# huggingface/parler-tts

Hardware: AMD Instinct MI355X
Metric: audio-seconds/sec (whole node) + p50 time-to-first-token, Mini-v1 bs=1/32 (higher is better)
Workload: dtype bf16; 1 GPU; parler-tts-mini-v1 bf16 bs=1/GPU greedy, 64 description + 32 prompt tokens, 860 frames = 9.985 s audio/utterance (868 decoder passes, hipGraph decode, DAC on-GPU); global_batch=1, frames=860, parallelism=utterance-sharded x1, weights broadcast once

## Files before the change

### parler_tts_amd/_native.py

```python
from __future__ import annotations

import ctypes as C
import os
from typing import Optional

PTTS_F32, PTTS_BF16 = 0, 1
PTTS_OK, PTTS_E_INVALID, PTTS_E_HIP, PTTS_E_MISSING, PTTS_E_CAPACITY, PTTS_E_UNSUPPORTED = 0, -1, -2, -3, -4, -5

_HERE = os.path.dirname(os.path.abspath(__file__))
LIB_PATH = os.path.join(_HERE, "libptts_hip.so")


class NativeLibraryError(RuntimeError):
    pass


class PttsConfig(C.Structure):
    _fields_ = [
        ("hidden_size", C.c_int32), ("num_layers", C.c_int32), ("num_heads", C.c_int32), ("ffn_dim", C.c_int32),
        ("num_codebooks", C.c_int32), ("vocab_size", C.c_int32), ("max_positions", C.c_int32), ("rope", C.c_int32),
        ("rope_theta", C.c_float), ("pad_token_id", C.c_int32), ("eos_token_id", C.c_int32), ("bos_token_id", C.c_int32),
        ("dtype", C.c_int32), ("max_batch", C.c_int32), ("max_ctx", C.c_int32), ("max_enc", C.c_int32),
        ("max_prompt", C.c_int32), ("device", C.c_int32), ("num_kv_heads", C.c_int32), ("num_cross_kv_heads", C.c_int32),
        ("weights_fp8", C.c_int32), ("kv_fp8", C.c_int32),
# ... 71 lines not shown
    "ptts_dac_debug_latents": (C.c_int, [_VP, C.POINTER(_VP)]),
    "ptts_t5_create": (C.c_int, [C.POINTER(PttsT5Config), C.POINTER(_VP)]),
    "ptts_t5_destroy": (None, [_VP]),
    "ptts_t5_load_weight": (C.c_int, [_VP, C.c_char_p, _VP, _I32, _I64P, _I32, _VP]),
    "ptts_t5_weights_ready": (C.c_int, [_VP]),
    "ptts_t5_encode": (C.c_int, [_VP, _VP, _VP, _I32, _I32, _VP, _VP]),
    "ptts_t5_relative_bucket": (C.c_int32, [_I32, _I32, _I32]),
    "ptts_t5_debug_graph_nodes": (C.c_int, [_VP, C.POINTER(_I32)]),
    "ptts_dac_debug_decode_upto": (C.c_int, [_VP, _VP, _I32, _I32, _I32, _VP, C.POINTER(_VP), C.POINTER(_I32), C.POINTER(_VP), C.POINTER(_I32), C.POINTER(_I32)]),
}

SESSION_SYMBOLS = {
    "ptts_admit_rows": (C.c_int, [_VP, _I32, C.POINTER(_I32), _VP, _VP, _VP, _VP, C.POINTER(_I32), _I32, C.POINTER(C.POINTER(PttsGenParams)), _VP]),
}

_lib: Optional[C.CDLL] = None


def load_library(path: Optional[str] = None) -> C.CDLL:
    global _lib
    if _lib is not None and path is None:
        return _lib
    import torch

    p = path or os.environ.get("PTTS_LIB", LIB_PATH)
    if not os.path.exists(p):
        raise NativeLibraryError(
            f"{p} not found: the HIP library is required (there is no CPU fallback). "
            "Build it with `python -c 'import __graft_entry__ as g; g.build()'`.")
    try:
        lib = C.CDLL(p)
    except OSError as e:
        raise NativeLibraryError(f"failed to load {p}: {e}") from e
    for name, (res, args) in list(SYMBOLS.items()) + list(SESSION_SYMBOLS.items()):
        try:
            fn = getattr(lib, name)
        except AttributeError as e:
            raise NativeLibraryError(f"{p} does not export {name}") from e
        fn.restype = res
        fn.argtypes = args
    if lib.ptts_abi_version() != ABI_VERSION:
        raise NativeLibraryError(f"ABI version mismatch: library {lib.ptts_abi_version()} != binding {ABI_VERSION}")
    if path is None:
        _lib = lib
    return lib


_hip: Optional[C.CDLL] = None

# ... 25 lines not shown
```

### parler_tts_amd/csrc/ptts_lm.hip

```cpp
#include <array>
#include <map>
#include <set>
#include <string>
#include <type_traits>
#include <vector>

#include "ptts_common.h"
#include "ptts_lm_kernels.h"
#include "ptts_gemv.h"
#include "ptts_strip_w8.h"
#include "ptts_gemm_launch.h"
#include "ptts_tail_launch.h"

thread_local std::string g_ptts_err;
int ptts_fail(int code, const char* fmt, ...) {
  char buf[1024];
  va_list ap;
  va_start(ap, fmt);
  vsnprintf(buf, sizeof(buf), fmt, ap);
  va_end(ap);
  g_ptts_err = buf;
  return code;
}
extern "C" const char* ptts_last_error(void) { return g_ptts_err.c_str(); }
// ... 61 lines not shown
  DevGen* gen = nullptr;
  ptts_gen_params gp;
  int B = 0, N = 0, P = 0;
  bool prefilled = false;
  bool h_ready = false;
  int lnproj = -1;
  int fuse_qa_max = 3;
  int last_graph_nodes = 0;
  bool fuse_qa = true;
  int fuse_x = -1;
  int fuse_x_nur = 2;
  float* xpart = nullptr;
  float* h2 = nullptr;
  bool fuse_xq = true;
  int lnproj_g = 0;
  int xattn_g = 0;
  bool xattn_g_ok = false;
  bool xattn_groups = true;
  int kv_ub = 0;
  int kv_bound = 0;
  std::map<long long, hipGraphExec_t> graphs;
  int* host_pinned = nullptr;
  bool session = false;
  int session_max_length = 0;
  int* row_maxlen = nullptr;
  SlotGen* slot_gen = nullptr;
  float* h_adm = nullptr;
  KvLayer* kv_layers_rows = nullptr;
  float* h_adm_rows = nullptr;
  AdmitMoveLayer* move_layers = nullptr;
// ... 53 lines not shown
}

inline void* at(void* p, size_t off) { return static_cast<char*>(p) + off; }

#ifdef PTTS_TIMING
#define PTTS_DBG_STAMP(args, on_, node_) (args).dbg = (e->dbg_stamps && (on_)) ? e->dbg_stamps + (node_) * 48 : nullptr
#else
#define PTTS_DBG_STAMP(args, on_, node_) do { } while (0)
#endif

int launch_status(const char* what) {
  hipError_t err = hipGetLastError();
  return err == hipSuccess ? PTTS_OK : ptts_fail(PTTS_E_HIP, "%s launch failed: %s", what, hipGetErrorString(err));
}

template <typename WT, int EPI>
int launch_lnproj(const ptts_engine* e, LnProjArgs p, hipStream_t st, int g) {
  constexpr int KT = Elem<WT>::KT;
  const int H = p.K;
  p.invK = 1.0f / (float)H;
  const int mg = p.M < g ? p.M : g;
  const size_t sh = (size_t)mg * (H * sizeof(WT) + 16) + 8 * 1024;
  const dim3 grid(p.N / 64, (p.M + g - 1) / g);
  const bool u16 = ((H / KT) / 2) % 16 == 0;
#define PTTS_LNPROJ_ONE(UW, NF4, G)                                                                                   \
  do {                                                                                                                \
    static PttsPerDeviceOnce attr_once;                                                                               \
    const int attr_dev = PttsPerDeviceOnce::device();                                                                 \
    if (sh > 64 * 1024 && attr_once.need(attr_dev)) {                                                                 \
      hipError_t ea = hipFuncSetAttribute(reinterpret_cast<const void*>(&lnproj_fused_kernel<WT, UW, NF4, G, EPI>),  \
                                          hipFuncAttributeMaxDynamicSharedMemorySize, 160 * 1024);                    \
      if (ea != hipSuccess) return ptts_fail(PTTS_E_HIP, "hipFuncSetAttribute(max dynamic LDS) failed: %s", hipGetErrorString(ea)); \
      attr_once.done(attr_dev);                                                                                       \
    }                                                                                                                 \
    ptts_klaunch(lnproj_fused_kernel<WT, UW, NF4, G, EPI>, grid, dim3(512), sh, st, p);                      \
  } while (0)
#define PTTS_LNPROJ_LAUNCH(UW, NF4)                                                                                   \
  do {                                                                                                                \
// ... 212 lines not shown

template <typename WT>
int strip_path(const ptts_engine* e, FwdView v, bool prefill, int Q, hipStream_t st) {
  const ptts_config& c = e->cfg;
  const int H = c.hidden_size, F = c.ffn_dim, nh = c.num_heads, B = v.B;
  const int nkv = e->nkv, nkc = e->nkc, Hkv = nkv * 64, QKV = H + 2 * Hkv;
  const int M = B * Q;
  const bool big = M > 8;
  const int dec = prefill ? 0 : 1;
  const float scale = 1.0f / sqrtf((float)(H / nh));
  const int S_used = prefill ? 1 : e->S_self;
  const bool lns = e->use_lns && !prefill && M > 8 && M <= 32;
  const int fo = (M > 8 && (!prefill || M <= 256)) ? 1 : 0;
  const int KT = Elem<WT>::KT;
  const int lnproj = e->lnproj >= 0 ? e->lnproj : 3;
  const int lnproj_g = e->lnproj_g > 0 ? e->lnproj_g : (M <= 40 ? 8 : 16);
  const bool lnproj_ok = lnproj > 0 && (!prefill || M <= 40) && M > 8 && !e->w8_strips && (H == 1024 || H == 1536) && ((H / KT) / 2) % 8 == 0 && QKV % 64 == 0 && F % 64 == 0;
  const int prefill_attn_mode = getenv("PTTS_PREFILL_ATTN") ? atoi(getenv("PTTS_PREFILL_ATTN")) : 3;
  const bool prefill_attn = prefill_attn_mode != 0;
  const bool kv_in_qkv = prefill && lnproj_ok && !c.rope && !e->L[0].ks_self;
  const bool kv_in_gemm = prefill && !kv_in_qkv && !lnproj_ok && M > 256 && !c.rope && !e->L[0].ks_self;
#define PTTS_DBG_BIG(args, l_, k_) PTTS_DBG_STAMP(args, !prefill && M > 8, (size_t)(l_) * 7 + (k_))
  for (int l = 0; l < c.num_layers; ++l) {
    const LayerW& w = e->L[l];
    void *const k_self = at(w.k_self, v.self_off), *const v_self = at(w.v_self, v.self_off);
    if (lnproj_ok) {
      LnProjArgs p = {};
      PTTS_DBG_BIG(p, l, 0);
      p.W = w.qkv; p.x = v.h; p.x_ld = H; p.gamma = w.ln1_g; p.beta = w.ln1_b; p.K = H; p.out = e->qkv; p.out_ld = QKV; p.M = M; p.N = QKV;
      if (kv_in_qkv) { p.kcache = k_self; p.vcache = v_self; p.kv_Q = Q; p.kv_cap = c.max_ctx; p.kv_heads = nkv; p.kv_H = H; }
      PTTS_TRY((launch_lnproj<WT, EPI_STORE>(e, p, st, lnproj_g)));
    } else {
      GemmArgs g = {}; g.decode = dec;
      g.W = w.qkv; g.W8 = w.qkv_p8; g.wscale = w.qkv_sc; g.x = v.h; g.x_ld = H; g.x_row_mul = 1; g.gamma = w.ln1_g; g.beta = w.ln1_b;
      g.out = e->qkv; g.out_ld = QKV; g.M = M; g.N = QKV; g.K = H; g.x_fo = fo;
      if (kv_in_gemm) { g.kcache = k_self; g.vcache = v_self; g.kv_rows_per_b = Q; g.kv_cap = c.max_ctx; g.nheads = nkv; g.kv_col0 = H; }
      PTTS_TRY((gemm_with_prologue<WT, PRO_LN, EPI_STORE>(e, g, st)));
    }
    if (prefill && !kv_in_qkv && !kv_in_gemm) {
      bool done8 = false;
      if constexpr (sizeof(WT) == 2) {
        if (w.ks_self) {
          hipLaunchKernelGGL((kv_append_kernel<WT, true>), dim3(Q, nkv, B), dim3(64), 0, st, e->qkv + H, e->qkv + H + Hkv, QKV, k_self, v_self, c.max_ctx,
                             Q, nkv, c.rope ? e->rope_cos : nullptr, c.rope ? e->rope_sin : nullptr, w.ks_self, w.vs_self);
          done8 = true;
        }
// ... 23 lines not shown
      }
    }
    if (!prefill && (M <= 8 || (e->xattn_groups && M <= 256)) && (H / KT) % 16 == 0 && (H == 512 || H == 1024 || H == 1536)) {
      XAttnArgs x = {};
      x.W = w.cq; x.x = v.h; x.x_ld = H; x.x_row_mul = 1; x.x_row_off = 0; x.gamma = w.ln2_g; x.beta = w.ln2_b; x.K = H;
      x.invK = 1.0f / (float)H; x.kcache = at(w.k_cross, v.cross_off); x.vcache = at(w.v_cross, v.cross_off); x.cap = c.max_enc; x.cur_len = v.cur_len; x.dims = e->dims;
      x.mask = v.enc_mask; x.mask_ld = c.max_enc; x.cos = c.rope ? e->rope_cos : nullptr; x.sin = c.rope ? e->rope_sin : nullptr;
      x.out = e->xw; x.B = M; x.nheads = nh; x.kv_heads = nkc; x.n_rep = nh / nkc; x.scale = scale; x.out_fo = fo;
      PTTS_DBG_BIG(x, l, 3);
      const int gsz = M <= 8 ? 8 : (e->xattn_g ? e->xattn_g : (e->xattn_g_ok ? (M <= 32 ? 2 : (M <= 64 ? 4 : 8)) : 8));
      launch_xattn_fused<WT>(x, gsz, st);
    } else {
    if (prefill && lnproj_ok) {
      LnProjArgs p = {};
      p.W = w.cq; p.x = v.h; p.x_ld = H; p.gamma = w.ln2_g; p.beta = w.ln2_b; p.K = H; p.out = e->qc; p.out_ld = H; p.M = M; p.N = H;
      PTTS_TRY((launch_lnproj<WT, EPI_STORE>(e, p, st, lnproj_g)));
    } else
    {
      GemmArgs g = {}; g.decode = dec;
      g.W = w.cq; g.x = v.h; g.x_ld = H; g.x_row_mul = 1; g.gamma = w.ln2_g; g.beta = w.ln2_b;
      g.out = e->qc; g.out_ld = H; g.M = M; g.N = H; g.K = H; g.x_fo = fo;
      if (lns) g.lnstat = e->lnstat;
      PTTS_TRY((gemm_with_prologue<WT, PRO_LN, EPI_STORE>(e, g, st)));
    }
    {
      AttnArgs a = cross_attn_args(e, v, w, Q, prefill, fo);
      a.hostP = v.P; a.hostN = v.N;
      if (prefill && prefill_attn) PTTS_TRY((launch_prefill_attn<WT>(a, B, st, prefill_attn_mode)));
      else PTTS_TRY((launch_attn<WT>(a, B, st, prefill ? 4 : e->cross_waves)));
    }
    }
// ... 6 lines not shown
      PTTS_TRY((launch_gemm<WT, PRO_COPY, EPI_RESID>(g, st)));
    }
    {
      GemmArgs g = {}; g.decode = dec;
      g.W = w.fc1; g.W8 = w.fc1_p8; g.wscale = w.fc1_sc; g.x = v.h; g.x_ld = H; g.x_row_mul = 1; g.gamma = w.ln3_g; g.beta = w.ln3_b;
      g.out_ld = F; g.M = M; g.N = F; g.K = H;
      GemmArgs g2 = {}; g2.decode = dec;
      g2.W = w.fc2; g2.W8 = w.fc2_p8; g2.wscale = w.fc2_sc; g2.x_ld = F; g2.x_row_mul = 1; g2.out = v.h; g2.out_ld = H; g2.M = M; g2.N = H; g2.K = F;
      if (big) {
        g.out = reinterpret_cast<float*>(e->xw2); g.x_fo = fo; g.out_fo = fo;
        if (lns) g.lnstat = e->lnstat;
        if (lnproj_ok && (lnproj >= 3 || (lnproj == 2 && M > 32))) {
          LnProjArgs p = {};
          p.W = w.fc1; p.x = v.h; p.x_ld = H; p.gamma = w.ln3_g; p.beta = w.ln3_b; p.K = H; p.out = e->xw2; p.out_ld = F; p.out_fo = fo; p.M = M; p.N = F;
          PTTS_DBG_BIG(p, l, 5);
          PTTS_TRY((launch_lnproj<WT, EPI_GELU_WT>(e, p, st, lnproj_g)));
        } else
        PTTS_TRY((gemm_with_prologue<WT, PRO_LN, EPI_GELU_WT>(e, g, st)));
        g2.x = reinterpret_cast<const float*>(e->xw2); g2.x_fo = fo;
        PTTS_DBG_BIG(g2, l, 6);
        PTTS_TRY((launch_gemm<WT, PRO_COPY, EPI_RESID>(g2, st)));
      } else {
        g.out = e->ffn;
        PTTS_TRY((launch_gemm<WT, PRO_LN, EPI_GELU>(g, st)));
        g2.x = e->ffn;
        PTTS_TRY((launch_gemm<WT, PRO_PLAIN, EPI_RESID>(g2, st)));
      }
    }
  }
  {
    GemmArgs g = {}; g.decode = dec;
// ... 109 lines not shown
           {"encoder_attn.out_proj.weight", w.co, w.co_rm, w.co_p8, w.co_sc, H, H, 0},
           {"fc1.weight", w.fc1, w.fc1_rm, w.fc1_p8, w.fc1_sc, F, H, 0},
           {"fc2.weight", w.fc2, w.fc2_rm, w.fc2_p8, w.fc2_sc, H, F, 0},
           {"self_attn_layer_norm.weight", w.ln1_g, nullptr, nullptr, nullptr, H, -1, 0}, {"self_attn_layer_norm.bias", w.ln1_b, nullptr, nullptr, nullptr, H, -1, 0},
           {"encoder_attn_layer_norm.weight", w.ln2_g, nullptr, nullptr, nullptr, H, -1, 0}, {"encoder_attn_layer_norm.bias", w.ln2_b, nullptr, nullptr, nullptr, H, -1, 0},
           {"final_layer_norm.weight", w.ln3_g, nullptr, nullptr, nullptr, H, -1, 0}, {"final_layer_norm.bias", w.ln3_b, nullptr, nullptr, nullptr, H, -1, 0}}};
}

void read_env_switches(ptts_engine* e) {
  if (const char* ev = getenv("PTTS_FUSE_X")) e->fuse_x = atoi(ev) ? 1 : 0;
  if (const char* ev = getenv("PTTS_FUSE_X_NUR")) { const int v = atoi(ev); if (v == 2 || v == 4) e->fuse_x_nur = v; }
  e->fuse_qa = !(getenv("PTTS_NO_FUSE_QA") && atoi(getenv("PTTS_NO_FUSE_QA")));
  if (const char* ev = getenv("PTTS_FUSE_QA_MAX")) e->fuse_qa_max = std::max(1, std::min(GV_MAX_ROWS, atoi(ev)));
  e->fuse_xq = !(getenv("PTTS_NO_FUSE_XQ") && atoi(getenv("PTTS_NO_FUSE_XQ")));
  if (const char* ev = getenv("PTTS_LNPROJ")) e->lnproj = std::max(0, std::min(3, atoi(ev)));
  if (const char* ev = getenv("PTTS_LNPROJ_G")) e->lnproj_g = atoi(ev) == 4 ? 4 : (atoi(ev) == 16 ? 16 : (atoi(ev) == 8 ? 8 : 0));
  if (const char* ev = getenv("PTTS_XATTN_G")) { const int g = atoi(ev); if (g == 2 || g == 4 || g == 8) e->xattn_g = e->xattn_g_ok ? g : 8; }
  e->xattn_groups = !(getenv("PTTS_NO_XATTN_GROUPS") && atoi(getenv("PTTS_NO_XATTN_GROUPS")));
}

hipStream_t pick_stream(ptts_engine*, void* s) { return reinterpret_cast<hipStream_t>(s); }

}

extern "C" int ptts_engine_create(const ptts_config* cfg, ptts_engine** out) {
  PTTS_CHECK(cfg && out, PTTS_E_INVALID, "null argument");
  const ptts_config& c = *cfg;
  PTTS_CHECK(c.hidden_size > 0 && c.num_heads > 0 && c.hidden_size % c.num_heads == 0, PTTS_E_INVALID, "hidden_size %d not divisible by num_heads %d", c.hidden_size, c.num_heads);
  PTTS_CHECK(c.hidden_size / c.num_heads == 64, PTTS_E_UNSUPPORTED, "head_dim must be 64 (Mini/Large v1), got %d", c.hidden_size / c.num_heads);
  PTTS_CHECK(c.dtype == PTTS_F32 || c.dtype == PTTS_BF16, PTTS_E_INVALID, "dtype must be PTTS_F32 or PTTS_BF16");
  PTTS_CHECK(c.hidden_size % 32 == 0 && c.ffn_dim % 32 == 0 && c.vocab_size % 16 == 0, PTTS_E_UNSUPPORTED,
// ... 135 lines not shown
  A(e->alloc(&e->qc, std::max(rows, enc_rows) * H));
  const size_t part_rows = std::max(rows * (size_t)e->S_self, (size_t)c.max_batch * 5) + 9;
  A(e->alloc(&e->part, part_rows * H));
  A(e->alloc(&e->stats, part_rows * nh * 2));
  A(e->alloc(&e->xpart, (size_t)nh * H));
  A(e->alloc(&e->h2, (size_t)H));
  A(e->alloc(&e->ffn, std::max(rows * F, rows * (size_t)H)));
  A(e->alloc(&e->logits, (size_t)c.max_batch * K * V));
  A(e->alloc(&e->sort_buf, 16));
  A(e->alloc_bytes(&e->xw, (rows + 16) * H * es));
  A(e->alloc_bytes(&e->xw2, std::max((rows + 16) * F, enc_rows * (size_t)H) * es));
  A(e->alloc(&e->lnstat, (size_t)c.max_batch * (H / 16) * 2 + 16));
  e->use_lns = H == 1024 || H == 1536;
  e->xattn_g_ok = (H == 1024 && ((H / (c.dtype == PTTS_BF16 ? 32 : 16)) / 2) % 16 == 0) || H == 1536;
  read_env_switches(e);
  A(e->alloc(&e->prefix, (size_t)c.max_batch * K * c.max_ctx));
  e->ids_ld = c.max_ctx + 8;
  A(e->alloc(&e->ids, (size_t)c.max_batch * K * e->ids_ld));
  A(e->alloc(&e->cur_len, c.max_batch)); A(e->alloc(&e->unfinished, (size_t)c.max_batch * K));
  A(e->alloc(&e->has_eos, (size_t)c.max_batch * K)); A(e->alloc(&e->first_unf, c.max_batch));
  A(e->alloc(&e->enc_mask, enc_rows + 64));
  A(e->alloc(&e->prompt_mask, rows));
  A(e->alloc(&e->dims, 1)); A(e->alloc(&e->gen, 1));
#undef A
  if (hipHostMalloc((void**)&e->host_pinned, ((size_t)c.max_batch * (K + 1) + 16) * 4) != hipSuccess) return fail(ptts_fail(PTTS_E_HIP, "hipHostMalloc failed"));
#ifdef PTTS_TIMING
  {
    const size_t n = (size_t)(c.num_layers + 1) * 7 * 48;
    rc = e->alloc(&e->dbg_stamps, n);
    if (rc != PTTS_OK) return fail(rc);
// ... 577 lines not shown
#ifdef PTTS_TIMING
extern "C" int ptts_debug_stamps(ptts_engine* e, long long** stamps_dev, int32_t* layers) {
  PTTS_CHECK(e && stamps_dev && layers, PTTS_E_INVALID, "null argument");
  *stamps_dev = e->dbg_stamps;
  *layers = e->cfg.num_layers;
  return PTTS_OK;
}
#endif

extern "C" int ptts_debug_graph_nodes(ptts_engine* e, int32_t* nodes) {
  PTTS_CHECK(e && nodes, PTTS_E_INVALID, "null argument");
  *nodes = e->last_graph_nodes;
  return PTTS_OK;
}

extern "C" int ptts_debug_hidden(ptts_engine* e, float** hidden_dev, int32_t* rows) {
  PTTS_CHECK(e && hidden_dev && rows, PTTS_E_INVALID, "null argument");
  *hidden_dev = e->h;
  *rows = e->B;
  return PTTS_OK;
}
```

### parler_tts_amd/csrc/ptts_lm_kernels.h

```cpp
#pragma once
#include "ptts_common.h"

struct DevDims {
  int P;
  int N;
  int max_length;
  int T_prefix;
  const long long* prefix;
  int prefix_ld;
};
struct DevGen {
  int max_length, min_new_tokens, do_sample, top_k, use_eos_gate;
  float temperature, top_p;
  unsigned long long seed;
};

template <typename ST> __device__ __forceinline__ float load_as_f32(const ST* p);
template <> __device__ __forceinline__ float load_as_f32<float>(const float* p) { return *p; }
template <> __device__ __forceinline__ float load_as_f32<bf16_t>(const bf16_t* p) { return bf16_to_f32(*p); }
template <typename DT> __device__ __forceinline__ void store_from_f32(DT* p, float v);
template <> __device__ __forceinline__ void store_from_f32<float>(float* p, float v) { *p = v; }
template <> __device__ __forceinline__ void store_from_f32<bf16_t>(bf16_t* p, float v) { *p = f32_to_bf16(v); }

template <typename WT, typename ST>
// ... 1785 lines not shown
  KDBG0(X)                                                                                                                              \
  KF(X, const void*, W)                                                                       \
  KF(X, const float*, x)                                                                               \
  KF(X, const float*, gamma) KF(X, const float*, beta) KF(X, void*, out)                                                              \
  KF(X, int, x_ld)                                                                                                                      \
  KF(X, int, K)                                                                                          \
  KF(X, int, M) KF(X, int, N) KTAIL(X, LnProjArgs)
struct LnProjArgs {
  PTTS_KMEMBERS(LnProjArgs)
  float invK;
  int out_ld;
  int out_fo;
  int kv_Q;
  void* kcache;
  void* vcache;
  int kv_cap, kv_heads, kv_H, kv_pad_;
  PTTS_DBG_FIELD
};
PTTS_KLAUNCH(LnProjArgs)

template <typename WT, int UW, int NF4, int G, int EPI>
__global__ void __launch_bounds__(512) lnproj_fused_kernel(PTTS_KPARAMS(LnProjArgs)) {
  PTTS_STAMP0();
  PTTS_KJOIN(LnProjArgs, a)
  constexpr int KT = Elem<WT>::KT, NWV = 8;
  static_assert(G <= 2 * NWV, "at most two rows per wave");
  extern __shared__ __attribute__((aligned(16))) char smem_raw[];
  const int lane = threadIdx.x & 63, wave = threadIdx.x >> 6;
  const int b0 = blockIdx.y * G, nb = min(G, a.M - b0), nbmax = min(G, a.M);
  const int row_bytes = a.K * (int)sizeof(WT) + 16;
  char* s_x = smem_raw;
  float* s_red = reinterpret_cast<float*>(smem_raw + (size_t)nbmax * row_bytes);
  const int nfrag = a.K / KT;
  const int strip = blockIdx.x * 4 + (wave >> 1);
  const int per = nfrag >> 1;
  const int t0 = (wave & 1) * per, t1 = t0 + per;
  const uint4* Wp = reinterpret_cast<const uint4*>(a.W) + (size_t)strip * nfrag * 64 + lane;
  const int q4 = lane >> 4, j = lane & 15;
  uint4 afr[UW];
  PTTS_WSTAMP(a, 0);
  if constexpr (G > NWV) {
    if (wave < nb) {
      const bool two = wave + NWV < nb;
      const float* xr0 = a.x + (size_t)(b0 + wave) * a.x_ld;
      const float* xr1 = a.x + (size_t)(b0 + (two ? wave + NWV : wave)) * a.x_ld;
      float4 v0[NF4], v1[NF4], g[NF4], bt[NF4];
#pragma unroll
      for (int i = 0; i < NF4; ++i) { v0[i] = *reinterpret_cast<const float4*>(xr0 + (lane + 64 * i) * 4); v1[i] = *reinterpret_cast<const float4*>(xr1 + (lane + 64 * i) * 4); }
#pragma unroll
      for (int i = 0; i < NF4; ++i) {
        g[i] = *reinterpret_cast<const float4*>(a.gamma + (lane + 64 * i) * 4);
        bt[i] = *reinterpret_cast<const float4*>(a.beta + (lane + 64 * i) * 4);
      }
      __builtin_amdgcn_sched_barrier(0);
      __builtin_amdgcn_s_barrier();
#pragma unroll
      for (int uu = 0; uu < UW; ++uu) afr[uu] = ld_nt16(Wp + (size_t)(t0 + uu) * 64);
      __builtin_amdgcn_sched_barrier(0);
      auto norm_row = [&](float4 (&v)[NF4], char* row) __attribute__((always_inline)) {
        const float c = __int_as_float(__builtin_amdgcn_readfirstlane(__float_as_int(v[0].x)));
        float s1 = 0.f, s2 = 0.f;
#pragma unroll
        for (int i = 0; i < NF4; ++i) {
          const float d0 = v[i].x - c, d1 = v[i].y - c, d2 = v[i].z - c, d3 = v[i].w - c;
          s1 += (d0 + d1) + (d2 + d3);
          s2 += (d0 * d0 + d1 * d1) + (d2 * d2 + d3 * d3);
        }
        s1 = wave_sum(s1);
        s2 = wave_sum(s2);
        const float dm = s1 * a.invK, mean = c + dm;
        const float rstd = rsqrtf(fmaxf(s2 * a.invK - dm * dm, 0.f) + 1e-5f);
#pragma unroll
        for (int i = 0; i < NF4; ++i)
          lds_store4<WT>(row, (lane + 64 * i) * 4, (v[i].x - mean) * rstd * g[i].x + bt[i].x, (v[i].y - mean) * rstd * g[i].y + bt[i].y,
                         (v[i].z - mean) * rstd * g[i].z + bt[i].z, (v[i].w - mean) * rstd * g[i].w + bt[i].w);
      };
      PTTS_WSTAMP(a, 1);
      norm_row(v0, s_x + (size_t)wave * row_bytes);
      if (two) norm_row(v1, s_x + (size_t)(wave + NWV) * row_bytes);
      PTTS_WSTAMP(a, 2);
    } else {
      __builtin_amdgcn_sched_barrier(0);
      __builtin_amdgcn_s_barrier();
#pragma unroll
      for (int uu = 0; uu < UW; ++uu) afr[uu] = ld_nt16(Wp + (size_t)(t0 + uu) * 64);
      __builtin_amdgcn_sched_barrier(0);
    }
  } else
  if (wave < nb) {
    const int m = b0 + wave;
    const float* xr = a.x + (size_t)m * a.x_ld;
    float4 v[NF4], g[NF4], bt[NF4];
#pragma unroll
    for (int i = 0; i < NF4; ++i) v[i] = *reinterpret_cast<const float4*>(xr + (lane + 64 * i) * 4);
#pragma unroll
    for (int i = 0; i < NF4; ++i) {
      g[i] = *reinterpret_cast<const float4*>(a.gamma + (lane + 64 * i) * 4);
      bt[i] = *reinterpret_cast<const float4*>(a.beta + (lane + 64 * i) * 4);
    }
    __builtin_amdgcn_sched_barrier(0);
    __builtin_amdgcn_s_barrier();
#pragma unroll
    for (int uu = 0; uu < UW; ++uu) afr[uu] = ld_nt16(Wp + (size_t)(t0 + uu) * 64);
    __builtin_amdgcn_sched_barrier(0);
    PTTS_WSTAMP(a, 1);
    const float c = __int_as_float(__builtin_amdgcn_readfirstlane(__float_as_int(v[0].x)));
    float s1 = 0.f, s2 = 0.f;
#pragma unroll
    for (int i = 0; i < NF4; ++i) {
      const float d0 = v[i].x - c, d1 = v[i].y - c, d2 = v[i].z - c, d3 = v[i].w - c;
      s1 += (d0 + d1) + (d2 + d3);
      s2 += (d0 * d0 + d1 * d1) + (d2 * d2 + d3 * d3);
    }
    s1 = wave_sum(s1);
    s2 = wave_sum(s2);
    const float dm = s1 * a.invK, mean = c + dm;
    const float rstd = rsqrtf(fmaxf(s2 * a.invK - dm * dm, 0.f) + 1e-5f);
    char* row = s_x + (size_t)wave * row_bytes;
#pragma unroll
    for (int i = 0; i < NF4; ++i)
      lds_store4<WT>(row, (lane + 64 * i) * 4, (v[i].x - mean) * rstd * g[i].x + bt[i].x, (v[i].y - mean) * rstd * g[i].y + bt[i].y,
                     (v[i].z - mean) * rstd * g[i].z + bt[i].z, (v[i].w - mean) * rstd * g[i].w + bt[i].w);
    PTTS_WSTAMP(a, 2);
  } else {
    __builtin_amdgcn_sched_barrier(0);
    __builtin_amdgcn_s_barrier();
#pragma unroll
    for (int uu = 0; uu < UW; ++uu) afr[uu] = ld_nt16(Wp + (size_t)(t0 + uu) * 64);
    __builtin_amdgcn_sched_barrier(0);
  }
  __syncthreads();
  PTTS_WSTAMP(a, 3);
  const char* brow = s_x + (size_t)min(j, nb - 1) * row_bytes + (size_t)q4 * 16;
  f32x4 acc = f32x4{0.f, 0.f, 0.f, 0.f}, acc2 = f32x4{0.f, 0.f, 0.f, 0.f};
  for (int tb = t0; tb < t1; tb += UW) {
    if (tb != t0) {
#pragma unroll
      for (int uu = 0; uu < UW; ++uu) afr[uu] = ld_nt16(Wp + (size_t)(tb + uu) * 64);
    }
#pragma unroll
    for (int uh = 0; uh < UW; uh += 8) {
      uint4 bfr[8];
#pragma unroll
      for (int uu = 0; uu < 8; ++uu) bfr[uu] = *reinterpret_cast<const uint4*>(brow + (size_t)(tb + uh + uu) * (KT * sizeof(WT)));
#pragma unroll
      for (int uu = 0; uu < 8; ++uu) {
        if (uu & 1) acc2 = MfmaStep<WT>::run(afr[uh + uu], bfr[uu], acc2);
        else acc = MfmaStep<WT>::run(afr[uh + uu], bfr[uu], acc);
      }
    }
  }
  PTTS_WSTAMP(a, 4);
  *reinterpret_cast<f32x4*>(s_red + ((size_t)wave * 64 + lane) * 4) = acc + acc2;
  __syncthreads();
  PTTS_WSTAMP(a, 5);
  if (wave < 4 && j < nb) {
    const f32x4 rr = *reinterpret_cast<const f32x4*>(s_red + ((size_t)(2 * wave) * 64 + lane) * 4) +
                     *reinterpret_cast<const f32x4*>(s_red + ((size_t)(2 * wave + 1) * 64 + lane) * 4);
    const int m = b0 + j, n = (blockIdx.x * 4 + wave) * 16 + q4 * 4;
    if (EPI == EPI_STORE) {
      *reinterpret_cast<float4*>(reinterpret_cast<float*>(a.out) + (size_t)m * a.out_ld + n) = make_float4(rr[0], rr[1], rr[2], rr[3]);
      if (a.kcache && n >= a.kv_H) {
        const int Hkv = a.kv_heads * 64, nn = n - a.kv_H, isv = nn >= Hkv, n2 = isv ? nn - Hkv : nn;
        const int head = n2 >> 6, d = n2 & 63, bu = m / a.kv_Q, pos = m - bu * a.kv_Q;
        WT* dst = reinterpret_cast<WT*>(isv ? a.vcache : a.kcache) + (((size_t)bu * a.kv_heads + head) * a.kv_cap + pos) * 64 + d;
#pragma unroll
        for (int e = 0; e < 4; ++e) store_from_f32<WT>(dst + e, rr[e]);
      }
    } else {
      act_store4<WT>(reinterpret_cast<WT*>(a.out), m, n, a.out_ld, a.out_fo, gelu_erf(rr[0]), gelu_erf(rr[1]), gelu_erf(rr[2]), gelu_erf(rr[3]));
    }
  }
}

template <typename WT, bool W8> struct RmRow {
  static __device__ __forceinline__ void ld8(const void* W, const float* sc, int row, int K, int k, float (&o)[8]) {
    if constexpr (W8) {
      const uint2 v = *reinterpret_cast<const uint2*>(reinterpret_cast<const uint8_t*>(W) + (size_t)row * K + k);
      const float s = sc[row];
      const auto a = __builtin_amdgcn_cvt_pk_f32_fp8((int)v.x, false), b = __builtin_amdgcn_cvt_pk_f32_fp8((int)v.x, true);
      const auto c = __builtin_amdgcn_cvt_pk_f32_fp8((int)v.y, false), d = __builtin_amdgcn_cvt_pk_f32_fp8((int)v.y, true);
      o[0] = a[0] * s; o[1] = a[1] * s; o[2] = b[0] * s; o[3] = b[1] * s; o[4] = c[0] * s; o[5] = c[1] * s; o[6] = d[0] * s; o[7] = d[1] * s;
    } else {
      const WT* p = reinterpret_cast<const WT*>(W) + (size_t)row * K + k;
#pragma unroll
      for (int e = 0; e < 8; ++e) o[e] = Elem<WT>::ld(p + e);
// ... 607 lines not shown
```

### parler_tts_amd/engine.py

```python
from __future__ import annotations

import ctypes as C
import math
from typing import Dict, Iterable, Optional, Tuple

import torch

from . import _native as N
from .quant import is_fp8_matrix


def _stream_ptr(stream: Optional["torch.cuda.Stream"] = None, device=None) -> C.c_void_p:
    s = stream if stream is not None else torch.cuda.current_stream(device)
    return C.c_void_p(s.cuda_stream)


def _shape_arr(t: torch.Tensor):
    return (C.c_int64 * t.dim())(*t.shape)


def rope_tables(head_dim: int, theta: float, num_positions: int) -> Tuple[torch.Tensor, torch.Tensor]:
    inv_freq = 1.0 / (theta ** (torch.arange(0, head_dim, 2, dtype=torch.int64).float() / head_dim))
    pos = torch.arange(num_positions, dtype=torch.int64).float()
    freqs = (inv_freq[:, None] @ pos[None, :]).transpose(0, 1)
# ... 113 lines not shown
        self.B, self.P = B, P
        self._keep = keep

    def first_token_sync(self):
        N.check(self.lib.ptts_first_token_sync(self._h), "ptts_first_token_sync")

    def first_token_times(self) -> Tuple[float, float]:
        pre, tail = C.c_float(), C.c_float()
        N.check(self.lib.ptts_first_token_times(self._h, C.byref(pre), C.byref(tail)), "ptts_first_token_times")
        return float(pre.value), float(tail.value)

    def graph_nodes(self) -> int:
        n = C.c_int32()
        N.check(self.lib.ptts_debug_graph_nodes(self._h, C.byref(n)), "ptts_debug_graph_nodes")
        return int(n.value)

    def set_audio_prefix(self, codes: Optional[torch.Tensor]):
        if codes is None or codes.shape[-1] == 0:
            N.check(self.lib.ptts_set_audio_prefix(self._h, C.c_void_p(), 1, 0, _stream_ptr(device=self.device)), "ptts_set_audio_prefix")
            return
        codes = codes.to(self.device, torch.int64).reshape(-1, codes.shape[-1]).contiguous()
        if codes.shape[0] % self.K:
            raise ValueError(f"audio prefix rows {codes.shape[0]} not a multiple of num_codebooks {self.K}")
        N.check(self.lib.ptts_set_audio_prefix(self._h, C.c_void_p(codes.data_ptr()), codes.shape[0] // self.K, codes.shape[1], _stream_ptr(device=self.device)),
                "ptts_set_audio_prefix")
        self._keep_prefix = codes

    def decode_steps(self, n: int):
        N.check(self.lib.ptts_decode_steps(self._h, int(n), _stream_ptr(device=self.device)), "ptts_decode_steps")

# ... 449 lines not shown
```

Measured before the change: 20.63 audio-seconds/sec.

## Make lnproj kernel loop over weight strips with CU-capped grid and prefetch

Reworks the fused LayerNorm+projection kernel so each block can walk several 64-row weight strips. When M exceeds 64, the grid's x dimension is capped at the CU count divided by the row groups, with tail strips spread evenly across blocks. The next strip's first weight fragments are prefetched before the barrier, and a double-buffered reduction area lets that overlap happen. It also adds min-waves hints to launch_bounds, makes the wave index uniform via readfirstlane, and reads the CU count at engine creation. A debug entry point is exposed to inspect the chosen grid. At small M the grid stays one strip per block, so the main effect there comes from the register and occupancy hints and the extra loop control.

```diff
diff --git a/include/ptts_debug.h b/include/ptts_debug.h
--- /dev/null
+++ b/include/ptts_debug.h
@@ -0,0 +1,14 @@
+#ifndef PTTS_DEBUG_H
+#define PTTS_DEBUG_H
+#include "ptts.h"
+#ifdef __cplusplus
+extern "C" {
+#endif
+
+int ptts_debug_lnproj_grid(ptts_engine* e, int32_t M, int32_t N, int32_t cus, int32_t passes, int32_t* grid_x, int32_t* grid_y,
+                           int32_t* full_passes, int32_t* tail_strips);
+
+#ifdef __cplusplus
+}
+#endif
+#endif
diff --git a/parler_tts_amd/_native.py b/parler_tts_amd/_native.py
--- a/parler_tts_amd/_native.py
+++ b/parler_tts_amd/_native.py
@@ -109,6 +109,10 @@
     "ptts_admit_rows": (C.c_int, [_VP, _I32, C.POINTER(_I32), _VP, _VP, _VP, _VP, C.POINTER(_I32), _I32, C.POINTER(C.POINTER(PttsGenParams)), _VP]),
 }
 
+DEBUG_SYMBOLS = {
+    "ptts_debug_lnproj_grid": (C.c_int, [_VP, _I32, _I32, _I32, _I32, C.POINTER(_I32), C.POINTER(_I32), C.POINTER(_I32), C.POINTER(_I32)]),
+}
+
 _lib: Optional[C.CDLL] = None
 
 
@@ -127,7 +131,7 @@
         lib = C.CDLL(p)
     except OSError as e:
         raise NativeLibraryError(f"failed to load {p}: {e}") from e
-    for name, (res, args) in list(SYMBOLS.items()) + list(SESSION_SYMBOLS.items()):
+    for name, (res, args) in list(SYMBOLS.items()) + list(SESSION_SYMBOLS.items()) + list(DEBUG_SYMBOLS.items()):
         try:
             fn = getattr(lib, name)
         except AttributeError as e:
diff --git a/parler_tts_amd/csrc/ptts_lm.hip b/parler_tts_amd/csrc/ptts_lm.hip
--- a/parler_tts_amd/csrc/ptts_lm.hip
+++ b/parler_tts_amd/csrc/ptts_lm.hip
@@ -99,6 +99,8 @@
   float* h2 = nullptr;
   bool fuse_xq = true;
   int lnproj_g = 0;
+  int lnproj_passes = 0;
+  int cus = 0;
   int xattn_g = 0;
   bool xattn_g_ok = false;
   bool xattn_groups = true;
@@ -182,14 +184,33 @@
   return err == hipSuccess ? PTTS_OK : ptts_fail(PTTS_E_HIP, "%s launch failed: %s", what, hipGetErrorString(err));
 }
 
+struct LnProjGrid { int g, gx, gy, full, tail; };
+LnProjGrid lnproj_grid(int M, int N, int cus, int g_forced, int passes_forced) {
+  LnProjGrid r;
+  r.g = g_forced > 0 ? g_forced : (M <= 40 ? 8 : 16);
+  r.gy = (M + r.g - 1) / r.g;
+  const int blocks = N / 64;
+  r.gx = blocks;
+  if (passes_forced > 0) r.gx = (blocks + passes_forced - 1) / passes_forced;
+  else if (M > 64) r.gx = std::max(1, cus / r.gy);
+  r.gx = std::max(1, std::min(r.gx, blocks));
+  r.full = blocks / r.gx;
+  const int rest = blocks - r.full * r.gx;
+  r.tail = (4 * rest + r.gx - 1) / r.gx;
+  return r;
+}
+
 template <typename WT, int EPI>
-int launch_lnproj(const ptts_engine* e, LnProjArgs p, hipStream_t st, int g) {
+int launch_lnproj(const ptts_engine* e, LnProjArgs p, hipStream_t st) {
   constexpr int KT = Elem<WT>::KT;
   const int H = p.K;
   p.invK = 1.0f / (float)H;
+  const LnProjGrid lg = lnproj_grid(p.M, p.N, e->cus, e->lnproj_g, e->lnproj_passes);
+  const int g = lg.g;
+  p.tail_strips = lg.tail;
   const int mg = p.M < g ? p.M : g;
-  const size_t sh = (size_t)mg * (H * sizeof(WT) + 16) + 8 * 1024;
-  const dim3 grid(p.N / 64, (p.M + g - 1) / g);
+  const size_t sh = (size_t)mg * (H * sizeof(WT) + 16) + (lg.full + (lg.tail > 0) > 1 ? 16 : 8) * 1024;
+  const dim3 grid(lg.gx, lg.gy);
   const bool u16 = ((H / KT) / 2) % 16 == 0;
 #define PTTS_LNPROJ_ONE(UW, NF4, G)                                                                                   \
   do {                                                                                                                \
@@ -432,7 +453,6 @@
   const int fo = (M > 8 && (!prefill || M <= 256)) ? 1 : 0;
   const int KT = Elem<WT>::KT;
   const int lnproj = e->lnproj >= 0 ? e->lnproj : 3;
-  const int lnproj_g = e->lnproj_g > 0 ? e->lnproj_g : (M <= 40 ? 8 : 16);
   const bool lnproj_ok = lnproj > 0 && (!prefill || M <= 40) && M > 8 && !e->w8_strips && (H == 1024 || H == 1536) && ((H / KT) / 2) % 8 == 0 && QKV % 64 == 0 && F % 64 == 0;
   const int prefill_attn_mode = getenv("PTTS_PREFILL_ATTN") ? atoi(getenv("PTTS_PREFILL_ATTN")) : 3;
   const bool prefill_attn = prefill_attn_mode != 0;
@@ -447,7 +467,7 @@
       PTTS_DBG_BIG(p, l, 0);
       p.W = w.qkv; p.x = v.h; p.x_ld = H; p.gamma = w.ln1_g; p.beta = w.ln1_b; p.K = H; p.out = e->qkv; p.out_ld = QKV; p.M = M; p.N = QKV;
       if (kv_in_qkv) { p.kcache = k_self; p.vcache = v_self; p.kv_Q = Q; p.kv_cap = c.max_ctx; p.kv_heads = nkv; p.kv_H = H; }
-      PTTS_TRY((launch_lnproj<WT, EPI_STORE>(e, p, st, lnproj_g)));
+      PTTS_TRY((launch_lnproj<WT, EPI_STORE>(e, p, st)));
     } else {
       GemmArgs g = {}; g.decode = dec;
       g.W = w.qkv; g.W8 = w.qkv_p8; g.wscale = w.qkv_sc; g.x = v.h; g.x_ld = H; g.x_row_mul = 1; g.gamma = w.ln1_g; g.beta = w.ln1_b;
@@ -501,7 +521,7 @@
     if (prefill && lnproj_ok) {
       LnProjArgs p = {};
       p.W = w.cq; p.x = v.h; p.x_ld = H; p.gamma = w.ln2_g; p.beta = w.ln2_b; p.K = H; p.out = e->qc; p.out_ld = H; p.M = M; p.N = H;
-      PTTS_TRY((launch_lnproj<WT, EPI_STORE>(e, p, st, lnproj_g)));
+      PTTS_TRY((launch_lnproj<WT, EPI_STORE>(e, p, st)));
     } else
     {
       GemmArgs g = {}; g.decode = dec;
@@ -538,7 +558,7 @@
           LnProjArgs p = {};
           p.W = w.fc1; p.x = v.h; p.x_ld = H; p.gamma = w.ln3_g; p.beta = w.ln3_b; p.K = H; p.out = e->xw2; p.out_ld = F; p.out_fo = fo; p.M = M; p.N = F;
           PTTS_DBG_BIG(p, l, 5);
-          PTTS_TRY((launch_lnproj<WT, EPI_GELU_WT>(e, p, st, lnproj_g)));
+          PTTS_TRY((launch_lnproj<WT, EPI_GELU_WT>(e, p, st)));
         } else
         PTTS_TRY((gemm_with_prologue<WT, PRO_LN, EPI_GELU_WT>(e, g, st)));
         g2.x = reinterpret_cast<const float*>(e->xw2); g2.x_fo = fo;
@@ -678,7 +698,10 @@
   if (const char* ev = getenv("PTTS_FUSE_QA_MAX")) e->fuse_qa_max = std::max(1, std::min(GV_MAX_ROWS, atoi(ev)));
   e->fuse_xq = !(getenv("PTTS_NO_FUSE_XQ") && atoi(getenv("PTTS_NO_FUSE_XQ")));
   if (const char* ev = getenv("PTTS_LNPROJ")) e->lnproj = std::max(0, std::min(3, atoi(ev)));
-  if (const char* ev = getenv("PTTS_LNPROJ_G")) e->lnproj_g = atoi(ev) == 4 ? 4 : (atoi(ev) == 16 ? 16 : (atoi(ev) == 8 ? 8 : 0));
+  if (const char* ev = getenv("PTTS_LNPROJ_G")) {
+    e->lnproj_g = atoi(ev) == 4 ? 4 : (atoi(ev) == 16 ? 16 : (atoi(ev) == 8 ? 8 : 0));
+    if (const char* cm = strchr(ev, ',')) e->lnproj_passes = std::max(0, std::min(64, atoi(cm + 1)));
+  }
   if (const char* ev = getenv("PTTS_XATTN_G")) { const int g = atoi(ev); if (g == 2 || g == 4 || g == 8) e->xattn_g = e->xattn_g_ok ? g : 8; }
   e->xattn_groups = !(getenv("PTTS_NO_XATTN_GROUPS") && atoi(getenv("PTTS_NO_XATTN_GROUPS")));
 }
@@ -844,6 +867,8 @@
   e->use_lns = H == 1024 || H == 1536;
   e->xattn_g_ok = (H == 1024 && ((H / (c.dtype == PTTS_BF16 ? 32 : 16)) / 2) % 16 == 0) || H == 1536;
   read_env_switches(e);
+  if (hipDeviceGetAttribute(&e->cus, hipDeviceAttributeMultiprocessorCount, c.device) != hipSuccess || e->cus < 1)
+    A(ptts_fail(PTTS_E_HIP, "hipDeviceGetAttribute(multiprocessor count) failed on device %d", c.device));
   A(e->alloc(&e->prefix, (size_t)c.max_batch * K * c.max_ctx));
   e->ids_ld = c.max_ctx + 8;
   A(e->alloc(&e->ids, (size_t)c.max_batch * K * e->ids_ld));
@@ -1451,6 +1476,15 @@
   return PTTS_OK;
 }
 
+extern "C" int ptts_debug_lnproj_grid(ptts_engine* e, int32_t M, int32_t N, int32_t cus, int32_t passes, int32_t* grid_x, int32_t* grid_y,
+                                      int32_t* full_passes, int32_t* tail_strips) {
+  PTTS_CHECK(grid_x && grid_y && full_passes && tail_strips, PTTS_E_INVALID, "null argument");
+  PTTS_CHECK(M >= 1 && N >= 64 && N % 64 == 0 && (e || cus >= 1), PTTS_E_INVALID, "M %d rows, N %d weight rows (a multiple of 64), %d compute units", M, N, cus);
+  const LnProjGrid g = e ? lnproj_grid(M, N, e->cus, e->lnproj_g, e->lnproj_passes) : lnproj_grid(M, N, cus, 0, passes);
+  *grid_x = g.gx; *grid_y = g.gy; *full_passes = g.full; *tail_strips = g.tail;
+  return PTTS_OK;
+}
+
 extern "C" int ptts_debug_hidden(ptts_engine* e, float** hidden_dev, int32_t* rows) {
   PTTS_CHECK(e && hidden_dev && rows, PTTS_E_INVALID, "null argument");
   *hidden_dev = e->h;
diff --git a/parler_tts_amd/csrc/ptts_lm_kernels.h b/parler_tts_amd/csrc/ptts_lm_kernels.h
--- a/parler_tts_amd/csrc/ptts_lm_kernels.h
+++ b/parler_tts_amd/csrc/ptts_lm_kernels.h
@@ -1823,30 +1823,36 @@
   int kv_Q;
   void* kcache;
   void* vcache;
-  int kv_cap, kv_heads, kv_H, kv_pad_;
+  int kv_cap, kv_heads, kv_H;
+  int tail_strips;
   PTTS_DBG_FIELD
 };
 PTTS_KLAUNCH(LnProjArgs)
 
+template <int UW, int NF4, int G> constexpr int lnproj_min_waves() { return (NF4 == 4 && !(UW == 16 && G == 16)) ? 4 : 2; }
 template <typename WT, int UW, int NF4, int G, int EPI>
-__global__ void __launch_bounds__(512) lnproj_fused_kernel(PTTS_KPARAMS(LnProjArgs)) {
+__global__ void __launch_bounds__(512, (lnproj_min_waves<UW, NF4, G>())) lnproj_fused_kernel(PTTS_KPARAMS(LnProjArgs)) {
   PTTS_STAMP0();
   PTTS_KJOIN(LnProjArgs, a)
   constexpr int KT = Elem<WT>::KT, NWV = 8;
   static_assert(G <= 2 * NWV, "at most two rows per wave");
   extern __shared__ __attribute__((aligned(16))) char smem_raw[];
-  const int lane = threadIdx.x & 63, wave = threadIdx.x >> 6;
+  const int lane = threadIdx.x & 63, wave = __builtin_amdgcn_readfirstlane(threadIdx.x >> 6);
   const int b0 = blockIdx.y * G, nb = min(G, a.M - b0), nbmax = min(G, a.M);
   const int row_bytes = a.K * (int)sizeof(WT) + 16;
   char* s_x = smem_raw;
   float* s_red = reinterpret_cast<float*>(smem_raw + (size_t)nbmax * row_bytes);
   const int nfrag = a.K / KT;
-  const int strip = blockIdx.x * 4 + (wave >> 1);
+  int sp = blockIdx.x * 4, cnt = 4;
   const int per = nfrag >> 1;
   const int t0 = (wave & 1) * per, t1 = t0 + per;
-  const uint4* Wp = reinterpret_cast<const uint4*>(a.W) + (size_t)strip * nfrag * 64 + lane;
+  const uint4* Wp = reinterpret_cast<const uint4*>(a.W) + (size_t)(sp + (wave >> 1)) * nfrag * 64 + lane;
   const int q4 = lane >> 4, j = lane & 15;
   uint4 afr[UW];
+  auto first_frags = [&]() __attribute__((always_inline)) {
+#pragma unroll
+    for (int uu = 0; uu < UW; ++uu) afr[uu] = ld_nt16(Wp + (size_t)(t0 + uu) * 64);
+  };
   PTTS_WSTAMP(a, 0);
   if constexpr (G > NWV) {
     if (wave < nb) {
@@ -1863,8 +1869,7 @@
       }
       __builtin_amdgcn_sched_barrier(0);
       __builtin_amdgcn_s_barrier();
-#pragma unroll
-      for (int uu = 0; uu < UW; ++uu) afr[uu] = ld_nt16(Wp + (size_t)(t0 + uu) * 64);
+      first_frags();
       __builtin_amdgcn_sched_barrier(0);
       auto norm_row = [&](float4 (&v)[NF4], char* row) __attribute__((always_inline)) {
         const float c = __int_as_float(__builtin_amdgcn_readfirstlane(__float_as_int(v[0].x)));
@@ -1891,8 +1896,7 @@
     } else {
       __builtin_amdgcn_sched_barrier(0);
       __builtin_amdgcn_s_barrier();
-#pragma unroll
-      for (int uu = 0; uu < UW; ++uu) afr[uu] = ld_nt16(Wp + (size_t)(t0 + uu) * 64);
+      first_frags();
       __builtin_amdgcn_sched_barrier(0);
     }
   } else
@@ -1909,8 +1913,7 @@
     }
     __builtin_amdgcn_sched_barrier(0);
     __builtin_amdgcn_s_barrier();
-#pragma unroll
-    for (int uu = 0; uu < UW; ++uu) afr[uu] = ld_nt16(Wp + (size_t)(t0 + uu) * 64);
+    first_frags();
     __builtin_amdgcn_sched_barrier(0);
     PTTS_WSTAMP(a, 1);
     const float c = __int_as_float(__builtin_amdgcn_readfirstlane(__float_as_int(v[0].x)));
@@ -1934,51 +1937,74 @@
   } else {
     __builtin_amdgcn_sched_barrier(0);
     __builtin_amdgcn_s_barrier();
-#pragma unroll
-    for (int uu = 0; uu < UW; ++uu) afr[uu] = ld_nt16(Wp + (size_t)(t0 + uu) * 64);
+    first_frags();
     __builtin_amdgcn_sched_barrier(0);
   }
   __syncthreads();
   PTTS_WSTAMP(a, 3);
   const char* brow = s_x + (size_t)min(j, nb - 1) * row_bytes + (size_t)q4 * 16;
-  f32x4 acc = f32x4{0.f, 0.f, 0.f, 0.f}, acc2 = f32x4{0.f, 0.f, 0.f, 0.f};
-  for (int tb = t0; tb < t1; tb += UW) {
-    if (tb != t0) {
-#pragma unroll
-      for (int uu = 0; uu < UW; ++uu) afr[uu] = ld_nt16(Wp + (size_t)(tb + uu) * 64);
-    }
-#pragma unroll
-    for (int uh = 0; uh < UW; uh += 8) {
-      uint4 bfr[8];
-#pragma unroll
-      for (int uu = 0; uu < 8; ++uu) bfr[uu] = *reinterpret_cast<const uint4*>(brow + (size_t)(tb + uh + uu) * (KT * sizeof(WT)));
-#pragma unroll
-      for (int uu = 0; uu < 8; ++uu) {
-        if (uu & 1) acc2 = MfmaStep<WT>::run(afr[uh + uu], bfr[uu], acc2);
-        else acc = MfmaStep<WT>::run(afr[uh + uu], bfr[uu], acc);
-      }
-    }
-  }
-  PTTS_WSTAMP(a, 4);
-  *reinterpret_cast<f32x4*>(s_red + ((size_t)wave * 64 + lane) * 4) = acc + acc2;
-  __syncthreads();
-  PTTS_WSTAMP(a, 5);
-  if (wave < 4 && j < nb) {
-    const f32x4 rr = *reinterpret_cast<const f32x4*>(s_red + ((size_t)(2 * wave) * 64 + lane) * 4) +
-                     *reinterpret_cast<const f32x4*>(s_red + ((size_t)(2 * wave + 1) * 64 + lane) * 4);
-    const int m = b0 + j, n = (blockIdx.x * 4 + wave) * 16 + q4 * 4;
-    if (EPI == EPI_STORE) {
-      *reinterpret_cast<float4*>(reinterpret_cast<float*>(a.out) + (size_t)m * a.out_ld + n) = make_float4(rr[0], rr[1], rr[2], rr[3]);
-      if (a.kcache && n >= a.kv_H) {
-        const int Hkv = a.kv_heads * 64, nn = n - a.kv_H, isv = nn >= Hkv, n2 = isv ? nn - Hkv : nn;
-        const int head = n2 >> 6, d = n2 & 63, bu = m / a.kv_Q, pos = m - bu * a.kv_Q;
-        WT* dst = reinterpret_cast<WT*>(isv ? a.vcache : a.kcache) + (((size_t)bu * a.kv_heads + head) * a.kv_cap + pos) * 64 + d;
-#pragma unroll
-        for (int e = 0; e < 4; ++e) store_from_f32<WT>(dst + e, rr[e]);
-      }
-    } else {
-      act_store4<WT>(reinterpret_cast<WT*>(a.out), m, n, a.out_ld, a.out_fo, gelu_erf(rr[0]), gelu_erf(rr[1]), gelu_erf(rr[2]), gelu_erf(rr[3]));
-    }
+  const int gx = gridDim.x, full = (a.N >> 6) / gx;
+  auto one_pass = [&](const int p) __attribute__((always_inline)) -> bool {
+    const bool act = (wave >> 1) < cnt;
+    f32x4 acc = f32x4{0.f, 0.f, 0.f, 0.f}, acc2 = f32x4{0.f, 0.f, 0.f, 0.f};
+    if (act) {
+      for (int tb = t0; tb < t1; tb += UW) {
+        if (tb != t0) {
+#pragma unroll
+          for (int uu = 0; uu < UW; ++uu) afr[uu] = ld_nt16(Wp + (size_t)(tb + uu) * 64);
+        }
+#pragma unroll
+        for (int uh = 0; uh < UW; uh += 8) {
+          uint4 bfr[8];
+#pragma unroll
+          for (int uu = 0; uu < 8; ++uu) bfr[uu] = *reinterpret_cast<const uint4*>(brow + (size_t)(tb + uh + uu) * (KT * sizeof(WT)));
+#pragma unroll
+          for (int uu = 0; uu < 8; ++uu) {
+            if (uu & 1) acc2 = MfmaStep<WT>::run(afr[uh + uu], bfr[uu], acc2);
+            else acc = MfmaStep<WT>::run(afr[uh + uu], bfr[uu], acc);
+          }
+        }
+      }
+    }
+    PTTS_WSTAMP(a, 4);
+    float* red = s_red + (p & 1) * (NWV * 64 * 4);
+    *reinterpret_cast<f32x4*>(red + ((size_t)wave * 64 + lane) * 4) = acc + acc2;
+    int nsp = (blockIdx.x + (p + 1) * gx) * 4, ncnt = 4;
+    if (p + 1 >= full) {
+      nsp = full * gx * 4 + blockIdx.x * a.tail_strips;
+      ncnt = p + 1 == full ? min(min(a.tail_strips, 4), (a.N >> 4) - nsp) : 0;
+    }
+    const bool more = ncnt > 0;
+    if (more && (wave >> 1) < ncnt) {
+      Wp = reinterpret_cast<const uint4*>(a.W) + (size_t)(nsp + (wave >> 1)) * nfrag * 64 + lane;
+      first_frags();
+      __builtin_amdgcn_sched_barrier(0);
+    }
+    __syncthreads();
+    PTTS_WSTAMP(a, 5);
+    if (wave < cnt && j < nb) {
+      const f32x4 rr = *reinterpret_cast<const f32x4*>(red + ((size_t)(2 * wave) * 64 + lane) * 4) +
+                       *reinterpret_cast<const f32x4*>(red + ((size_t)(2 * wave + 1) * 64 + lane) * 4);
+      const int m = b0 + j, n = (sp + wave) * 16 + q4 * 4;
+      if (EPI == EPI_STORE) {
+        *reinterpret_cast<float4*>(reinterpret_cast<float*>(a.out) + (size_t)m * a.out_ld + n) = make_float4(rr[0], rr[1], rr[2], rr[3]);
+        if (a.kcache && n >= a.kv_H) {
+          const int Hkv = a.kv_heads * 64, nn = n - a.kv_H, isv = nn >= Hkv, n2 = isv ? nn - Hkv : nn;
+          const int head = n2 >> 6, d = n2 & 63, bu = m / a.kv_Q, pos = m - bu * a.kv_Q;
+          WT* dst = reinterpret_cast<WT*>(isv ? a.vcache : a.kcache) + (((size_t)bu * a.kv_heads + head) * a.kv_cap + pos) * 64 + d;
+#pragma unroll
+          for (int e = 0; e < 4; ++e) store_from_f32<WT>(dst + e, rr[e]);
+        }
+      } else {
+        act_store4<WT>(reinterpret_cast<WT*>(a.out), m, n, a.out_ld, a.out_fo, gelu_erf(rr[0]), gelu_erf(rr[1]), gelu_erf(rr[2]), gelu_erf(rr[3]));
+      }
+    }
+    sp = nsp;
+    cnt = ncnt;
+    return more;
+  };
+  if (one_pass(0)) {
+    for (int p = 1; one_pass(p); ++p) {}
   }
 }
 
diff --git a/parler_tts_amd/engine.py b/parler_tts_amd/engine.py
--- a/parler_tts_amd/engine.py
+++ b/parler_tts_amd/engine.py
@@ -151,6 +151,11 @@
         n = C.c_int32()
         N.check(self.lib.ptts_debug_graph_nodes(self._h, C.byref(n)), "ptts_debug_graph_nodes")
         return int(n.value)
+
+    def lnproj_grid(self, rows: int, weight_rows: int) -> Tuple[int, int, int, int]:
+        out = [C.c_int32() for _ in range(4)]
+        N.check(self.lib.ptts_debug_lnproj_grid(self._h, rows, weight_rows, 0, 0, *[C.byref(o) for o in out]), "ptts_debug_lnproj_grid")
+        return tuple(int(o.value) for o in out)
 
     def set_audio_prefix(self, codes: Optional[torch.Tensor]):
         if codes is None or codes.shape[-1] == 0:
```

Result: no change. 20.58 audio-seconds/sec (-0.3%).
